# Yusheng-Xu/VGS-SVGS-Segmentation

Measured on AMD Instinct MI355X. Metric: segmented points/sec (end-to-end VGS), higher is better.
Workload: dtype f32

## Files before the change

include/vgs.h:

```cpp
#ifndef VGS_H_
#define VGS_H_

#include <stdint.h>

#ifdef __cplusplus
extern "C" {
#endif

typedef enum {
  VGS_OK = 0,
  VGS_E_ARG = 1,
  VGS_E_STATE = 2,
  VGS_E_HIP = 3,
  VGS_E_NOMEM = 4,
  VGS_E_UNSUPPORTED = 5,
  VGS_E_IO = 6,
  VGS_E_PEER = 7
} vgs_status;

typedef struct {
  int32_t method;
  float voxel_size;
  float graph_size;
  float sig_p, sig_n, sig_o, sig_e, sig_c, sig_w;
// ... 47 lines not shown
vgs_status vgs_commit_points(vgs_ctx* ctx);
vgs_status vgs_host_alloc(void** p, uint64_t bytes);
vgs_status vgs_host_free(void* p);
vgs_status vgs_host_register(void* p, uint64_t bytes);
vgs_status vgs_host_unregister(void* p);

vgs_status vgs_voxelize(vgs_ctx* ctx);
vgs_status vgs_features(vgs_ctx* ctx);
vgs_status vgs_adjacency(vgs_ctx* ctx);
vgs_status vgs_segment(vgs_ctx* ctx);
vgs_status vgs_run(vgs_ctx* ctx);

vgs_status svgs_set_supervoxel_labels(vgs_ctx* ctx, const int32_t* labels_host, int32_t max_label);
vgs_status svgs_supervoxels(vgs_ctx* ctx);
vgs_status svgs_segment(vgs_ctx* ctx);
vgs_status svgs_get_supervoxel_labels(vgs_ctx* ctx, int32_t* labels, int32_t* max_label);

vgs_status vgs_get_counts(vgs_ctx* ctx, int64_t* counts );
vgs_status vgs_get_stage_times(vgs_ctx* ctx, double* ms );
vgs_status vgs_get_schedule_counters(vgs_ctx* ctx, int64_t* out );
vgs_status vgs_get_schedule_counters_ex(vgs_ctx* ctx, int64_t* out, int32_t n);
vgs_status vgs_screen_table(const vgs_params* params, float* d2_stop, float* ctab_scale, float* ctab );
vgs_status vgs_get_bbox(vgs_ctx* ctx, double* min3_max3);
vgs_status vgs_get_voxel_table(vgs_ctx* ctx, uint32_t* key, int32_t* start, int32_t* point_idx);
vgs_status vgs_get_voxel_centers(vgs_ctx* ctx, float* center3V);
vgs_status vgs_get_point_voxel(vgs_ctx* ctx, int32_t* voxel_of_point );
vgs_status vgs_get_attributes(vgs_ctx* ctx, float* centroid, float* normal, float* eigen8, uint8_t* used);
vgs_status vgs_get_lists(vgs_ctx* ctx, int32_t which, int64_t* offsets, int32_t* idx);
enum { VGS_ORDER_VOXEL_ID = 0, VGS_ORDER_REFERENCE = 1 };
vgs_status vgs_get_lists_ordered(vgs_ctx* ctx, int32_t which, int32_t order, int64_t* offsets, int32_t* idx);
vgs_status vgs_get_adjacency_counts(vgs_ctx* ctx, int32_t* n_all );
vgs_status vgs_get_local_weights(vgs_ctx* ctx, int32_t node_id, int32_t* n, int32_t* ids, float* weights);
vgs_status vgs_get_node_labels(vgs_ctx* ctx, int32_t* component_root ,
                               int32_t* kept_label );
vgs_status vgs_get_point_labels(vgs_ctx* ctx, int32_t* labels );
vgs_status vgs_get_point_labels_async(vgs_ctx* ctx, int32_t* labels);
vgs_status vgs_wait_point_labels(vgs_ctx* ctx);
vgs_status vgs_get_point_labels_device(vgs_ctx* ctx, const int32_t** labels_dev );
vgs_status vgs_get_clusters(vgs_ctx* ctx, int64_t* offsets, int32_t* point_idx);
vgs_status vgs_get_clusters_ordered(vgs_ctx* ctx, int32_t order, int64_t* offsets, int32_t* point_idx);
vgs_status vgs_get_clusters_device(vgs_ctx* ctx, const int64_t** offsets_dev, const int32_t** point_idx_dev);
vgs_status vgs_get_segment_descriptors(vgs_ctx* ctx, int64_t* n_points, int32_t* n_nodes, float* bbox6, double* centroid3, double* cov6,
                                       double* evals3, double* evecs9, float* eigen8);
vgs_status vgs_get_segment_descriptors_device(vgs_ctx* ctx, const int64_t** n_points, const int32_t** n_nodes, const float** bbox6,
                                              const double** centroid3, const double** cov6, const double** evals3, const double** evecs9,
                                              const float** eigen8);
// ... 43 lines not shown
```

vgs-svgs-segmentation_amd/_lib.py:

```python
from __future__ import annotations

import ctypes as C
import os
import subprocess

_HERE = os.path.dirname(os.path.abspath(__file__))
LIB_PATH = os.path.join(_HERE, os.path.basename(os.environ.get("VGS_LIB", "libvgs_hip.so")))
CSRC = os.path.join(_HERE, "csrc")

VGS_OK, VGS_E_ARG, VGS_E_STATE, VGS_E_HIP, VGS_E_NOMEM, VGS_E_UNSUPPORTED, VGS_E_IO, VGS_E_PEER = range(8)
STATUS_NAMES = ["VGS_OK", "VGS_E_ARG", "VGS_E_STATE", "VGS_E_HIP", "VGS_E_NOMEM", "VGS_E_UNSUPPORTED", "VGS_E_IO", "VGS_E_PEER"]

N_POINTS, N_FINITE, N_VOXELS, N_USED, N_ADJ, N_CLUSTERS, N_KEPT, N_PAIRS, N_DEPTH, N_ISOLATED, N_REATTACHED, N_SUPERVOXELS = range(12)
N_COUNTS = 16
T_VOXELIZE, T_FEATURES, T_ADJACENCY, T_LOCALCUT, T_MERGE, T_LABELS, T_TOTAL, T_LOCALCUT_KERNEL, T_SUPERVOXEL = range(9)
T_COUNT = 12


class VgsParams(C.Structure):
    _fields_ = [
        ("method", C.c_int32), ("voxel_size", C.c_float), ("graph_size", C.c_float),
        ("sig_p", C.c_float), ("sig_n", C.c_float), ("sig_o", C.c_float), ("sig_e", C.c_float), ("sig_c", C.c_float),
        ("sig_w", C.c_float), ("cut_thred", C.c_float),
        ("points_min", C.c_int32), ("adjacency_min", C.c_int32), ("voxels_min", C.c_int32),
# ... 24 lines not shown
    ("vgs_set_points", C.c_int, [_P, _P, C.c_int64, C.c_int32]),
    ("vgs_set_points_device", C.c_int, [_P, _P, C.c_int64, C.c_int32]),
    ("vgs_stage_points", C.c_int, [_P, _P, C.c_int64, C.c_int32]),
    ("vgs_commit_points", C.c_int, [_P]),
    ("vgs_host_alloc", C.c_int, [C.POINTER(_P), C.c_uint64]),
    ("vgs_host_free", C.c_int, [_P]),
    ("vgs_host_register", C.c_int, [_P, C.c_uint64]),
    ("vgs_host_unregister", C.c_int, [_P]),
    ("vgs_voxelize", C.c_int, [_P]),
    ("vgs_features", C.c_int, [_P]),
    ("vgs_adjacency", C.c_int, [_P]),
    ("vgs_segment", C.c_int, [_P]),
    ("vgs_run", C.c_int, [_P]),
    ("svgs_set_supervoxel_labels", C.c_int, [_P, _P, C.c_int32]),
    ("svgs_supervoxels", C.c_int, [_P]),
    ("svgs_segment", C.c_int, [_P]),
    ("svgs_get_supervoxel_labels", C.c_int, [_P, _P, C.POINTER(C.c_int32)]),
    ("vgs_get_counts", C.c_int, [_P, _P]),
    ("vgs_get_schedule_counters", C.c_int, [_P, _P]),
    ("vgs_get_schedule_counters_ex", C.c_int, [_P, _P, C.c_int32]),
    ("vgs_screen_table", C.c_int, [_P, _P, _P, _P]),
    ("vgs_get_stage_times", C.c_int, [_P, _P]),
    ("vgs_get_bbox", C.c_int, [_P, _P]),
    ("vgs_get_voxel_table", C.c_int, [_P, _P, _P, _P]),
    ("vgs_get_voxel_centers", C.c_int, [_P, _P]),
    ("vgs_get_point_voxel", C.c_int, [_P, _P]),
    ("vgs_get_attributes", C.c_int, [_P, _P, _P, _P, _P]),
    ("vgs_get_lists", C.c_int, [_P, C.c_int32, _P, _P]),
    ("vgs_get_lists_ordered", C.c_int, [_P, C.c_int32, C.c_int32, _P, _P]),
    ("vgs_get_adjacency_counts", C.c_int, [_P, _P]),
    ("vgs_get_local_weights", C.c_int, [_P, C.c_int32, C.POINTER(C.c_int32), _P, _P]),
    ("vgs_get_node_labels", C.c_int, [_P, _P, _P]),
    ("vgs_get_point_labels", C.c_int, [_P, _P]),
    ("vgs_get_point_labels_async", C.c_int, [_P, _P]),
    ("vgs_wait_point_labels", C.c_int, [_P]),
    ("vgs_get_point_labels_device", C.c_int, [_P, C.POINTER(_P)]),
    ("vgs_get_clusters", C.c_int, [_P, _P, _P]),
    ("vgs_get_clusters_ordered", C.c_int, [_P, C.c_int32, _P, _P]),
    ("vgs_get_clusters_device", C.c_int, [_P, _P, _P]),
    ("vgs_get_segment_descriptors", C.c_int, [_P, _P, _P, _P, _P, _P, _P, _P, _P]),
    ("vgs_get_segment_descriptors_device", C.c_int, [_P, _P, _P, _P, _P, _P, _P, _P, _P]),
    ("vgs_get_own_segment_moments", C.c_int, [_P, C.c_int64, _P, _P, _P, _P, _P, _P, _P]),
    ("vgs_segment_descriptors_from_moments", C.c_int, [_P, C.c_int64, _P, _P, _P, _P, _P, _P, _P, _P, _P, _P, _P, _P, _P]),
    ("vgs_get_segment_boxes", C.c_int, [_P, C.c_int32, _P, _P, _P, _P, _P]),
    ("vgs_get_segment_boxes_device", C.c_int, [_P, C.c_int32, _P, _P, _P, _P, _P]),
    ("vgs_get_own_segment_extents", C.c_int, [_P, C.c_int64, C.c_int32, _P, _P, _P, _P, _P, _P, _P]),
# ... 45 lines not shown
```

vgs-svgs-segmentation_amd/api.py:

```python
from __future__ import annotations

import ctypes as C

import numpy as np

from . import _lib
from ._lib import VgsError, VgsGridState, VgsParams


def default_params(method=2, **kw):
    p = VgsParams()
    L = _lib.lib()
    (L.vgs_params_default_svgs if method == 3 else L.vgs_params_default_vgs)(C.byref(p))
    for k, v in kw.items():
        if not hasattr(p, k):
            raise AttributeError(k)
        setattr(p, k, v)
    return p


def parse_task_file(path):
    p = VgsParams()
    a = C.create_string_buffer(512)
    b = C.create_string_buffer(512)
# ... 97 lines not shown
        self._ck(self._L.vgs_get_counts(self._h, _ptr(c)))
        names = ["points", "finite", "voxels", "used", "adj", "clusters", "kept", "pairs", "depth", "isolated", "reattached",
                 "supervoxels", "handed_over", "class_a", "class_bc", "class_d"]
        return {k: int(c[i]) for i, k in enumerate(names)}

    def schedule_counters(self):
        c = np.zeros(13, dtype=np.int64)
        self._ck(self._L.vgs_get_schedule_counters_ex(self._h, _ptr(c), 13))
        names = ("lazy_gave_up", "list_overflow", "handed_over", "dense_sent_on", "handed_over_large", "outside_limits", "cross_put_off", "banded",
                 "extra_large", "pair_list_cut", "pair_list_entries", "voted_over", "pair_list_pool_full")
        return dict(zip(names, (int(x) for x in c)))

    def stage_times(self):
        t = np.zeros(_lib.T_COUNT, dtype=np.float64)
        self._ck(self._L.vgs_get_stage_times(self._h, _ptr(t)))
        names = ["voxelize", "features", "adjacency", "localcut", "merge", "labels", "total", "localcut_kernel", "supervoxel", "localcut_bulk"]
        return {k: float(t[i]) for i, k in enumerate(names)}

    def bbox(self):
        b = np.zeros(6, dtype=np.float64)
        self._ck(self._L.vgs_get_bbox(self._h, _ptr(b)))
        return b

    def voxel_table(self):
        c = self.counts()
        V, nf = c["voxels"], c["finite"]
        key = np.zeros((V, 3), dtype=np.uint32)
        start = np.zeros(V + 1, dtype=np.int32)
        pidx = np.zeros(nf, dtype=np.int32)
        self._ck(self._L.vgs_get_voxel_table(self._h, _ptr(key), _ptr(start), _ptr(pidx)))
        return dict(key=key, start=start, point_idx=pidx)

    def voxel_centers(self):
        V = self.counts()["voxels"]
        c = np.zeros((V, 3), dtype=np.float32)
        self._ck(self._L.vgs_get_voxel_centers(self._h, _ptr(c)))
        return c

    def point_voxel(self):
        out = np.zeros(self.n, dtype=np.int32)
        self._ck(self._L.vgs_get_point_voxel(self._h, _ptr(out)))
        return out

    def attributes(self):
        V = self.counts()["voxels"]
        cen = np.zeros((V, 3), dtype=np.float32)
# ... 328 lines not shown
```

vgs-svgs-segmentation_amd/csrc/capi.hip:

```cpp
#include <algorithm>
#include <cstdio>
#include <cstdlib>
#include <cstring>
#include <fstream>
#include <string>
#include <vector>

#include <dlfcn.h>

#include "vgs_context.hpp"

static thread_local std::string g_create_err;

static const char* const VGS_STAGE_NAMES[VGS_T_COUNT] = {"vgs:voxelize", "vgs:features", "vgs:adjacency", "vgs:localcut", "vgs:merge", "vgs:labels",
                                                         "vgs:total", "vgs:localcut_kernel", "vgs:supervoxels", "vgs:localcut_bulk", "", ""};
struct RoctxApi {
  int (*push)(const char*) = nullptr;
  int (*pop)() = nullptr;
  RoctxApi() {
    for (const char* name : {"librocprofiler-sdk-roctx.so.1", "librocprofiler-sdk-roctx.so", "libroctx64.so.4", "libroctx64.so"}) {
      void* h = dlopen(name, RTLD_LAZY | RTLD_LOCAL);
      if (!h) continue;
      push = (int (*)(const char*))dlsym(h, "roctxRangePushA");
      pop = (int (*)())dlsym(h, "roctxRangePop");
// ... 206 lines not shown
  if (c->ev_ho) (void)hipEventDestroy(c->ev_ho);
  if (c->ev_ho2) (void)hipEventDestroy(c->ev_ho2);
  if (c->ev_d2h) (void)hipEventDestroy(c->ev_d2h);
  delete c;
}

vgs_status vgs_set_params(vgs_ctx* c, const vgs_params* p) {
  if (!c || !p) return VGS_E_ARG;
  if (!(p->voxel_size > 0.f) || !(p->graph_size > 0.f) || !(p->sig_w != 0.f)) { c->err = "vgs_set_params: voxel_size, graph_size > 0, sig_w != 0"; return VGS_E_ARG; }
  if (p->method != c->P.method || p->device != c->P.device) { c->err = "vgs_set_params: method and device are fixed at vgs_create"; return VGS_E_ARG; }
  if (p->vccs_mode != 0 && p->vccs_mode != 1) { c->err = "vgs_set_params: vccs_mode must be 0 (synchronous variant) or 1 (PCL's order)"; return VGS_E_ARG; }
  int keep = ST_SEGMENTED;
  const vgs_params& o = c->P;
  if (p->cut_thred != o.cut_thred || p->sig_p != o.sig_p || p->sig_n != o.sig_n || p->sig_o != o.sig_o || p->sig_e != o.sig_e ||
      p->sig_c != o.sig_c || p->sig_w != o.sig_w || p->adjacency_min != o.adjacency_min || p->voxels_min != o.voxels_min ||
      p->q7_count_as_index != o.q7_count_as_index)
    keep = ST_ADJACENCY;
  if (p->graph_size != o.graph_size) keep = ST_FEATURES;
  if (p->points_min != o.points_min) keep = ST_VOXELS;
  if (p->voxel_size != o.voxel_size || p->seed_size != o.seed_size || p->color_impt != o.color_impt ||
      p->spatial_impt != o.spatial_impt || p->normal_impt != o.normal_impt || p->vccs_mode != o.vccs_mode)
    keep = ST_POINTS;
  if (c->stage > keep) c->stage = keep;
  if (keep < ST_SEGMENTED) { c->sd_valid = false; c->sb_valid[0] = c->sb_valid[1] = false; c->sg_valid = false; c->sg_halo_valid = false; c->sg_own_K = -1; }
  if (keep == ST_POINTS && c->P.method == 3 && !c->sv_labels_external) { c->sv_have_labels = false; c->sv_max_label = 0; c->sv_label_n = -1; }
  c->P = *p;
  return VGS_OK;
}

const char* vgs_last_error_string(const vgs_ctx* c) { return c ? c->err.c_str() : g_create_err.c_str(); }

static vgs_status set_points_common(vgs_ctx* c, int64_t n, int32_t stride_bytes) {
  if (n < 0 || (stride_bytes != 12 && stride_bytes != 16)) { c->err = "set_points: n >= 0 and stride_bytes 12 or 16 required"; return VGS_E_ARG; }
  if (n >= (int64_t)1 << 31) { c->err = "set_points: more than 2^31-1 points"; return VGS_E_UNSUPPORTED; }
  c->N = n;
  c->stride_f = stride_bytes / 4;
  c->stage = ST_POINTS;
  c->sd_valid = false;
  c->sb_valid[0] = c->sb_valid[1] = false;
  c->sg_valid = false; c->sg_halo_valid = false; c->sg_own_K = -1;
  c->grid_covers = false;
  c->counts[VGS_N_POINTS] = n;
  for (int i = 0; i < VGS_T_COUNT; ++i) { c->times[i] = 0; c->tev_pending[i] = false; }
  c->sv_have_labels = false; c->sv_labels_external = false; c->sv_max_label = 0; c->sv_label_n = -1;
  c->n_own = -1; c->own_first = 0;
  return VGS_OK;
// ... 187 lines not shown
    VGS_HIP_TRY(c, hipMemcpy(ev.data(), c->evals.p, ev.size() * 4, hipMemcpyDeviceToHost));
    int64_t tot = 0;
    for (uint32_t x : ev) tot += x;
    c->counts[VGS_N_PAIRS] = tot;
  }
  for (int i = 0; i < VGS_N_COUNTS; ++i) counts[i] = c->counts[i];
  return VGS_OK;
}

vgs_status vgs_get_stage_times(vgs_ctx* c, double* ms) {
  if (!c || !ms) return VGS_E_ARG;
  { vgs_status sr = vgs_resolve_times(c); if (sr != VGS_OK) return sr; }
  if (c->P.method == 2 && c->stage >= ST_SEGMENTED)
    c->times[VGS_T_TOTAL] = c->times[VGS_T_VOXELIZE] + c->times[VGS_T_FEATURES] + c->times[VGS_T_ADJACENCY] + c->times[VGS_T_LOCALCUT] + c->times[VGS_T_MERGE];
  for (int i = 0; i < VGS_T_COUNT; ++i) ms[i] = c->times[i];
  return VGS_OK;
}

vgs_status vgs_get_schedule_counters(vgs_ctx* c, int64_t* out) { return vgs_get_schedule_counters_ex(c, out, 8); }

vgs_status vgs_get_schedule_counters_ex(vgs_ctx* c, int64_t* out, int32_t n) {
  if (!c || !out || n < 0 || n > 16) return VGS_E_ARG;
  for (int i = 0; i < n; ++i) out[i] = c->lc_diag[i];
  return VGS_OK;
}

vgs_status vgs_get_bbox(vgs_ctx* c, double* b) {
  if (!c || !b) return VGS_E_ARG;
  if (c->stage < ST_VOXELS) { c->err = "vgs_get_bbox: voxelize first"; return VGS_E_STATE; }
  for (int a = 0; a < 3; ++a) { b[a] = c->box.min[a]; b[3 + a] = c->box.max[a]; }
  return VGS_OK;
}

vgs_status vgs_get_voxel_table(vgs_ctx* c, uint32_t* key, int32_t* start, int32_t* point_idx) {
  if (!c) return VGS_E_ARG;
  if (c->stage < ST_VOXELS) { c->err = "vgs_get_voxel_table: voxelize first"; return VGS_E_STATE; }
  VGS_HIP_TRY(c, hipSetDevice(c->device));
  if (key && c->V > 0) {
    std::vector<uint64_t> code((size_t)c->V);
    VGS_HIP_TRY(c, hipMemcpy(code.data(), c->vox_code.p, code.size() * 8, hipMemcpyDeviceToHost));
    for (int64_t v = 0; v < c->V; ++v) {
      key[3 * v + 0] = vm_compact21(code[v] >> 2);
      key[3 * v + 1] = vm_compact21(code[v] >> 1);
      key[3 * v + 2] = vm_compact21(code[v]);
    }
  }
// ... 291 lines not shown
```

vgs-svgs-segmentation_amd/csrc/multigpu.hip:

```cpp
#include <algorithm>
#include <cstring>
#include <vector>

#include <rocprim/rocprim.hpp>

#include "vgs_context.hpp"

__global__ void k_point_sources(const uint32_t* __restrict__ perm, const uint32_t* __restrict__ pt_vox, int64_t nf, int64_t own_first, int64_t n_own,
                                int64_t V, uint8_t* __restrict__ mix) {
  int64_t j = (int64_t)blockIdx.x * blockDim.x + threadIdx.x;
  if (j >= nf) return;
  const uint32_t v = pt_vox[j];
  const int64_t i = (int64_t)perm[j];
  if (v != 0xffffffffu) mix[((i >= own_first && i < own_first + n_own) ? 0 : V) + v] = 1;
}

__global__ void k_owned(const uint64_t* __restrict__ vox_code, int64_t V, float res_f, float min_x, float min_y, double lo_x, double lo_y,
                        double hi_x, double hi_y, uint8_t* __restrict__ owned, uint8_t* __restrict__ straddle, const uint8_t* __restrict__ mix, double near) {
  int64_t v = (int64_t)blockIdx.x * blockDim.x + threadIdx.x;
  if (v >= V) return;
  const uint64_t code = vox_code[v];
  const double cx = (double)vm_voxel_center(vm_compact21(code >> 2), res_f, min_x);
  const double cy = (double)vm_voxel_center(vm_compact21(code >> 1), res_f, min_y);
  owned[v] = (cx >= lo_x && cx < hi_x && cy >= lo_y && cy < hi_y) ? 1 : 0;
// ... 237 lines not shown
vgs_status vgs_grid_advance(vgs_ctx* c, vgs_grid_state* g) {
  if (!c || !g) return VGS_E_ARG;
  if (c->stage < ST_POINTS) { c->err = "vgs_grid_advance: no input cloud"; return VGS_E_STATE; }
  VGS_HIP_TRY(c, hipSetDevice(c->device));
  OctreeBox box;
  box_from_state(g, (double)c->P.voxel_size, box);
  const bool was_pinned = c->grid_pinned;
  c->grid_pinned = false;
  vgs_status st = vgs_grow_box_from(c, box, false);
  c->grid_pinned = was_pinned;
  if (st != VGS_OK) return st;
  g->defined = box.defined ? 1 : 0;
  g->depth = box.depth;
  for (int a = 0; a < 3; ++a) { g->min[a] = box.min[a]; g->shift[a] = box.shift[a]; }
  return VGS_OK;
}

vgs_status vgs_set_grid(vgs_ctx* c, const vgs_grid_state* g) {
  if (!c || !g) return VGS_E_ARG;
  if (!g->defined) { c->err = "vgs_set_grid: undefined grid state"; return VGS_E_ARG; }
  box_from_state(g, (double)c->P.voxel_size, c->box);
  c->grid_pinned = true;
  c->grid_covers = false;
  if (c->stage > ST_POINTS) c->stage = ST_POINTS;
  return VGS_OK;
}

vgs_status vgs_set_grid_covering(vgs_ctx* c, const vgs_grid_state* g) {
  vgs_status s = vgs_set_grid(c, g);
  if (s == VGS_OK) c->grid_covers = true;
  return s;
}

vgs_status vgs_set_owned_region(vgs_ctx* c, const double* lo, const double* hi) {
  if (!c || !lo || !hi) return VGS_E_ARG;
  c->own_lo[0] = lo[0]; c->own_lo[1] = lo[1]; c->own_hi[0] = hi[0]; c->own_hi[1] = hi[1];
  c->have_region = true;
  if (c->stage > ST_ADJACENCY) c->stage = ST_ADJACENCY;
  return VGS_OK;
}

vgs_status vgs_set_own_point_range(vgs_ctx* c, int64_t first, int64_t n_own) {
  if (!c || n_own < -1 || first < 0) return VGS_E_ARG;
  c->own_first = first;
  c->n_own = n_own;
  if (c->stage > ST_ADJACENCY) c->stage = ST_ADJACENCY;
// ... 187 lines not shown
```

vgs-svgs-segmentation_amd/csrc/vgs_context.hpp:

```cpp
#ifndef VGS_CONTEXT_HPP_
#define VGS_CONTEXT_HPP_

#include <hip/hip_runtime.h>
#include <stdint.h>
#include <string.h>

#include <string>
#include <vector>

#include "../../include/vgs.h"
#include "vgs_math.h"
#include "pairlist.hpp"

typedef VgsNode NodeRec;
static_assert(sizeof(NodeRec) == 64, "NodeRec must be 64 bytes");

#ifdef __HIPCC__
__device__ __forceinline__ int64_t vgs_xcd_item(unsigned int b, int64_t n) {
  const int64_t per = (n + 7) >> 3;
  return (int64_t)(b & 7u) * per + (int64_t)(b >> 3);
}
#endif
static inline unsigned int vgs_xcd_grid(int64_t n) { return (unsigned int)(((n + 7) >> 3) << 3); }

// ... 90 lines not shown

  const float* xyz = nullptr;
  DevBuf<float> xyz_buf[2];
  int xyz_cur = 0;
  hipStream_t s_h2d = nullptr, s_d2h = nullptr;
  hipEvent_t ev_h2d = nullptr, ev_d2h = nullptr;
  hipEvent_t ev_rb = nullptr;
  bool gathered = false;
  bool bricks_ready = false;
  bool staged = false;
  int64_t staged_n = 0;
  int staged_stride = 12;
  bool pt_labels_pending = false;
  bool labels_event_valid = false;
  bool d2h_open = false;
  const int32_t* d2h_src = nullptr;
  int64_t N = 0;
  int stride_f = 3;

  OctreeBox box;
  bool grid_pinned = false;
  bool grid_covers = false;
  int n_epochs = 0;

  DevBuf<uint64_t> code_a, code_b;
  DevBuf<uint32_t> perm_a, perm_b;
  DevBuf<uint8_t> sort_tmp;
  DevBuf<uint64_t> grow_state;
  DevBuf<uint32_t> pt_vox;
  DevBuf<uint32_t> vox_tile;
  DevBuf<uint32_t> head_flag;
  DevBuf<uint64_t> vox_code;
  DevBuf<uint32_t> vox_start;
  DevBuf<float> xs, ys, zs;
  int64_t Nf = 0;
  int64_t V = 0;
  int code_bits = 0;

  DevBuf<NodeRec> node;
  DevBuf<uint32_t> used_ids, used_rank;
  int64_t U = 0;

  DevBuf<uint64_t> hkey;
  DevBuf<uint32_t> hval;
  uint32_t hbits = 0;
  DevBuf<int32_t> offsets;
// ... 219 lines not shown
```

vgs-svgs-segmentation_amd/csrc/voxelize.hip:

```cpp
#include <cstddef>
#include <cstdlib>
#include <cstring>
#include <string.h>

#include <rocprim/rocprim.hpp>

#include <algorithm>
#include <cmath>
#include <limits>

#include "vgs_context.hpp"

bool OctreeBox::contains(const float* p) const {
  if (!defined) return false;
  for (int a = 0; a < 3; ++a)
    if ((double)p[a] < min[a] || (double)p[a] >= max[a]) return false;
  return true;
}

void OctreeBox::adopt(const float* p) {
  const double eps = (double)std::numeric_limits<float>::epsilon();
  while (true) {
    if (!defined) {
      for (int a = 0; a < 3; ++a) { min[a] = (double)p[a] - res / 2; max[a] = (double)p[a] + res / 2; }
// ... 15 lines not shown
      any = any || hi[a] || ((double)p[a] < min[a]);
    }
    if (!any) return;
    double side = (double)(1u << depth) * res;
    for (int a = 0; a < 3; ++a)
      if (!hi[a]) { min[a] -= side; shift[a] += (1ull << depth); }
    depth++;
    side = (double)(1u << depth) * res - eps;
    for (int a = 0; a < 3; ++a) max[a] = min[a] + side;
  }
}

__device__ __forceinline__ bool finite3(float x, float y, float z) {
  return (vm_bits(x) & 0x7f800000u) != 0x7f800000u && (vm_bits(y) & 0x7f800000u) != 0x7f800000u &&
         (vm_bits(z) & 0x7f800000u) != 0x7f800000u;
}

struct GrowState {
  double min[3], max[3], res;
  unsigned long long shift[3];
  unsigned long long found;
  long long start;
  int depth, defined, done, n_epochs, record, overflow;
  Epoch epochs[VGS_MAX_EPOCHS];
};

struct BoxD { double min[3], max[3]; int defined; };
__device__ __forceinline__ bool fv_outside(float x, float y, float z, const BoxD& g) {
  if (!finite3(x, y, z)) return false;
  return !g.defined || (double)x < g.min[0] || (double)x >= g.max[0] || (double)y < g.min[1] ||
         (double)y >= g.max[1] || (double)z < g.min[2] || (double)z >= g.max[2];
}

__global__ void k_first_violation(const float* __restrict__ xyz, int stride_f, int64_t n, GrowState* __restrict__ gs) {
  if (gs->done) return;
  BoxD box;
  for (int a = 0; a < 3; ++a) { box.min[a] = gs->min[a]; box.max[a] = gs->max[a]; }
  box.defined = gs->defined;
  unsigned long long* result = &gs->found;
  const int64_t start = gs->start;
  unsigned long long best = ~0ull;
  const int64_t tid = (int64_t)blockIdx.x * blockDim.x + threadIdx.x;
  const int64_t nthreads = box.defined ? (int64_t)gridDim.x * blockDim.x : (int64_t)8 * blockDim.x;
  if (tid >= nthreads) return;
  if (stride_f == 3 && (((uintptr_t)xyz) & 15u) == 0) {
    const float4* q = (const float4*)xyz;
// ... 93 lines not shown
    unsigned long long best = ~0ull;
    for (int64_t i = start + tid; i < n_prefix; i += 1024) {
      const float* p = xyz + i * stride_f;
      if (fv_outside(p[0], p[1], p[2], box)) { best = (unsigned long long)i; break; }
    }
    for (int o = 32; o > 0; o >>= 1) { const unsigned long long other = __shfl_down(best, o, 64); best = other < best ? other : best; }
    __syncthreads();
    if ((tid & 63) == 0) s_best[tid >> 6] = best;
    __syncthreads();
    if (tid == 0) {
      unsigned long long b = ~0ull;
      for (int w = 0; w < 16; ++w) b = s_best[w] < b ? s_best[w] : b;
      if (b == ~0ull) { if (S.start < n_prefix) S.start = n_prefix; S.found = ~0ull; s_best[0] = 0ull; }
      else if (pinned) { S.done = 2; s_best[0] = 0ull; }
      else { grow_adopt(xyz, stride_f, &S, b); s_best[0] = (S.done || S.overflow) ? 0ull : 1ull; }
    }
    __syncthreads();
    if (s_best[0] == 0ull) break;
    __syncthreads();
  }
  for (int k = tid; k < (int)(sizeof(GrowState) / 8); k += 1024) ((unsigned long long*)gs)[k] = ((const unsigned long long*)&S)[k];
}

template <typename KeyT>
__global__ void k_make_codes(const float* __restrict__ xyz, int stride_f, int64_t n, const GrowState* __restrict__ gs,
                             double res, int code_bits, KeyT* __restrict__ code, uint32_t* __restrict__ perm, int pack_shift) {
  int64_t i = (int64_t)blockIdx.x * blockDim.x + threadIdx.x;
  if (i >= n) return;
  const float* p = xyz + i * stride_f;
  float x = p[0], y = p[1], z = p[2];
  uint64_t c = 0;
  if (finite3(x, y, z)) {
    int e = gs->n_epochs - 1;
    while (e > 0 && i < gs->epochs[e].first) --e;
    const Epoch& ep = gs->epochs[e];
    uint32_t kx = vm_axis_key(x, ep.min[0], res) + (uint32_t)(gs->shift[0] - ep.shift[0]);
    uint32_t ky = vm_axis_key(y, ep.min[1], res) + (uint32_t)(gs->shift[1] - ep.shift[1]);
    uint32_t kz = vm_axis_key(z, ep.min[2], res) + (uint32_t)(gs->shift[2] - ep.shift[2]);
    c = (1ull << code_bits) | vm_morton(kx, ky, kz);
  }
  if (pack_shift > 0) { code[i] = (KeyT)((c << pack_shift) | (uint64_t)i); return; }
  code[i] = (KeyT)c;
  perm[i] = (uint32_t)i;
}

#define VR_TB 512
#define VR_KPT 4
#define VR_TILE (VR_TB * VR_KPT)

template <typename KeyT>
__device__ __forceinline__ void vr_load(const KeyT* __restrict__ code, int64_t n, int64_t j0, KeyT (&k)[VR_KPT], KeyT& prev) {
  struct alignas(sizeof(KeyT) * VR_KPT) Vec { KeyT v[VR_KPT]; };
  if (j0 + VR_KPT <= n) {
    const Vec q = *(const Vec*)(code + j0);
#pragma unroll
    for (int i = 0; i < VR_KPT; ++i) k[i] = q.v[i];
// ... 102 lines not shown
  if (j0 >= n) return;
  uint32_t out[VR_KPT];
#pragma unroll
  for (int i = 0; i < VR_KPT; ++i) {
    if ((m >> i) & 1u) { vox_code[run] = c[i] & mask; vox_start[run] = (uint32_t)(j0 + i); ++run; }
    out[i] = c[i] != 0 ? run - 1u : 0xffffffffu;
  }
  if (j0 + VR_KPT <= n) {
    *(uint4*)(pt_vox + j0) = make_uint4(out[0], out[1], out[2], out[3]);
  } else {
#pragma unroll
    for (int i = 0; i < VR_KPT; ++i) if (j0 + i < n) pt_vox[j0 + i] = out[i];
  }
}

__global__ void k_gather_points(const float* __restrict__ xyz, int stride_f, const uint32_t* __restrict__ perm, int64_t nf,
                                float* __restrict__ xs, float* __restrict__ ys, float* __restrict__ zs) {
  int64_t j = (int64_t)blockIdx.x * blockDim.x + threadIdx.x;
  if (j >= nf) return;
  const float* p = xyz + (int64_t)perm[j] * stride_f;
  xs[j] = p[0]; ys[j] = p[1]; zs[j] = p[2];
}

vgs_status vgs_grow_box_from(vgs_ctx* c, OctreeBox& box, bool record_epochs) {
  static_assert(sizeof(GrowState) % 8 == 0, "GrowState is copied as 64-bit words");
  VGS_HIP_TRY(c, c->counters.ensure(64));
  VGS_HIP_TRY(c, c->grow_state.ensure(sizeof(GrowState) / 8));
  GrowState* d_g = (GrowState*)c->grow_state.p;
  static thread_local GrowState h;
  std::memset(&h, 0, sizeof(h));
  for (int a = 0; a < 3; ++a) { h.min[a] = box.min[a]; h.max[a] = box.max[a]; h.shift[a] = box.shift[a]; }
  h.res = box.res; h.depth = box.depth; h.defined = box.defined ? 1 : 0;
  h.found = ~0ull; h.start = 0; h.record = record_epochs ? 1 : 0;
  const size_t hb_bytes = offsetof(GrowState, epochs) + sizeof(Epoch);
  const bool covering = c->grid_pinned && c->grid_covers && record_epochs && box.defined;
  if (covering) h.done = 1;
  if (record_epochs && box.defined) {
    Epoch& e = h.epochs[h.n_epochs++];
    e.first = 0;
    for (int a = 0; a < 3; ++a) { e.min[a] = box.min[a]; e.shift[a] = box.shift[a]; }
  }
  {
    const size_t hb = hb_bytes;
    static_assert(offsetof(GrowState, epochs) + sizeof(Epoch) <= 1024, "the growth header fits its slot of the pinned scratch");
    const void* src = &h;
    if (c->pin) { memcpy((char*)c->pin + 1024, &h, hb); src = (char*)c->pin + 1024; }
    VGS_HIP_TRY(c, hipMemcpyAsync(d_g, src, hb, hipMemcpyHostToDevice, c->stream));
  }
  if (covering) {
    c->n_epochs = h.n_epochs;
    return VGS_OK;
  }
  const int pinned = (c->grid_pinned && record_epochs) ? 1 : 0;
  const int blocks = (int)std::max<int64_t>(8, std::min<int64_t>((c->N / 4 + 255) / 256 + 1, (int64_t)c->K.fv_blocks));
  hipLaunchKernelGGL(k_grow_prefix, dim3(1), dim3(1024), 0, c->stream, c->xyz, c->stride_f, std::min<int64_t>(c->N, 8192), d_g, pinned);
  for (int batch = 0; batch < 64; ++batch) {
    for (int k = 0; k < (batch == 0 ? 2 : 8); ++k) {
      hipLaunchKernelGGL(k_first_violation, dim3(blocks), dim3(256), 0, c->stream, c->xyz, c->stride_f, c->N, d_g);
      hipLaunchKernelGGL(k_adopt, dim3(1), dim3(1), 0, c->stream, c->xyz, c->stride_f, d_g, pinned);
    }
    VGS_READBACK(c, &h, d_g, offsetof(GrowState, epochs));
    if (h.done) break;
  }
  if (h.done == 2) { c->err = "a point lies outside the pinned grid"; return VGS_E_ARG; }
  if (h.overflow || !h.done) { c->err = "octree grew more than VGS_MAX_EPOCHS times"; return VGS_E_UNSUPPORTED; }
  for (int a = 0; a < 3; ++a) { box.min[a] = h.min[a]; box.max[a] = h.max[a]; box.shift[a] = h.shift[a]; }
  box.depth = h.depth; box.defined = h.defined != 0;
  if (record_epochs) c->n_epochs = h.n_epochs;
  return VGS_OK;
}

static vgs_status grow_box(vgs_ctx* c) {
  if (!c->grid_pinned) {
    c->box = OctreeBox();
    c->box.res = (double)c->P.voxel_size;
  }
  return vgs_grow_box_from(c, c->box, true);
}

template <typename KeyT>
static vgs_status voxelize_sorted_table(vgs_ctx* c) {
  const int64_t N = c->N;
  const int TB = 256;
  const unsigned nb = (unsigned)((N + TB - 1) / TB);
  KeyT* code_a = (KeyT*)c->code_a.p;
  KeyT* code_b = (KeyT*)c->code_b.p;
  const unsigned key_bits = (unsigned)(c->code_bits + 1);
  int idx_bits = 1;
  while (idx_bits < 32 && ((int64_t)1 << idx_bits) < N) ++idx_bits;
  const int pack_shift = (sizeof(KeyT) == 8 && (int)key_bits + idx_bits <= 64) ? idx_bits : 0;
  hipLaunchKernelGGL((k_make_codes<KeyT>), dim3(nb), dim3(TB), 0, c->stream, c->xyz, c->stride_f, N, (const GrowState*)c->grow_state.p, c->box.res,
                     c->code_bits, code_a, c->perm_a.p, pack_shift);

  using nine_bits = rocprim::radix_sort_config<rocprim::default_config, rocprim::default_config,
                                               rocprim::radix_sort_onesweep_config<rocprim::kernel_config<1024, 6>, rocprim::kernel_config<1024, 6>, 9,
                                                                                   rocprim::block_radix_rank_algorithm::match>>;
  const bool use9 = (key_bits + 8) / 9 < (key_bits + 7) / 8;
  auto sort_pairs = [&](void* tmp, size_t& bytes) -> hipError_t {
    if (pack_shift > 0)
      return use9 ? rocprim::radix_sort_keys_desc<nine_bits>(tmp, bytes, code_a, code_b, (size_t)N, (unsigned)pack_shift, (unsigned)pack_shift + key_bits, c->stream)
                  : rocprim::radix_sort_keys_desc(tmp, bytes, code_a, code_b, (size_t)N, (unsigned)pack_shift, (unsigned)pack_shift + key_bits, c->stream);
    return use9 ? rocprim::radix_sort_pairs_desc<nine_bits>(tmp, bytes, code_a, code_b, c->perm_a.p, c->perm_b.p, (size_t)N, 0, key_bits, c->stream)
                : rocprim::radix_sort_pairs_desc(tmp, bytes, code_a, code_b, c->perm_a.p, c->perm_b.p, (size_t)N, 0, key_bits, c->stream);
  };
  size_t tmp_bytes = 0;
  VGS_HIP_TRY(c, sort_pairs(nullptr, tmp_bytes));
  VGS_HIP_TRY(c, c->sort_tmp.ensure(tmp_bytes));
  VGS_HIP_TRY(c, sort_pairs(c->sort_tmp.p, tmp_bytes));
  const int64_t n_tiles = (N + VR_TILE - 1) / VR_TILE;
  VGS_HIP_TRY(c, c->vox_tile.ensure((size_t)(2 * n_tiles)));
  uint32_t* tile_heads = c->vox_tile.p;
  uint32_t* tile_valid = c->vox_tile.p + n_tiles;
  unsigned long long* d_cnt = (unsigned long long*)c->counters.p;
  hipLaunchKernelGGL((k_run_counts<KeyT>), dim3((unsigned)n_tiles), dim3(VR_TB), 0, c->stream, code_b, N, pack_shift, c->perm_b.p, tile_heads, tile_valid);
  hipLaunchKernelGGL(k_tile_offsets, dim3(1), dim3(1024), 0, c->stream, tile_heads, tile_valid, n_tiles, d_cnt);
  unsigned long long h2[2] = {0, 0};
  if (vgs_can_split_readback(c)) {
    { vgs_status sb = vgs_readback_begin(c, d_cnt, sizeof(h2)); if (sb != VGS_OK) return sb; }
    VGS_HIP_TRY(c, c->xs.ensure(N + 1)); VGS_HIP_TRY(c, c->ys.ensure(N + 1)); VGS_HIP_TRY(c, c->zs.ensure(N + 1));
    hipLaunchKernelGGL(k_gather_points, dim3(nb), dim3(TB), 0, c->stream, c->xyz, c->stride_f, c->perm_b.p, N, c->xs.p, c->ys.p, c->zs.p);
    c->gathered = true;
    { vgs_status se = vgs_readback_end(c, h2, sizeof(h2)); if (se != VGS_OK) return se; }
  } else {
    VGS_READBACK(c, h2, d_cnt, sizeof(h2));
  }
  const unsigned long long nf = h2[0];
  const uint32_t v_total = (uint32_t)h2[1];
  c->Nf = (int64_t)nf;
  c->V = (int64_t)v_total;
  VGS_HIP_TRY(c, c->vox_code.ensure(c->V + 1)); VGS_HIP_TRY(c, c->vox_start.ensure(c->V + 1));
  const uint64_t mask = (c->code_bits >= 64) ? ~0ull : ((1ull << c->code_bits) - 1ull);
  hipLaunchKernelGGL((k_voxel_runs<KeyT>), dim3((unsigned)n_tiles), dim3(VR_TB), 0, c->stream, code_b, N, pack_shift, tile_heads, mask, c->pt_vox.p,
                     c->vox_code.p, c->vox_start.p, v_total, (uint32_t)c->Nf);
  return VGS_OK;
}

vgs_status vgs_stage_voxelize(vgs_ctx* c) {
  const int64_t N = c->N;
  c->V = 0; c->Nf = 0; c->U = 0;
  vgs_status st = grow_box(c);
  if (st != VGS_OK) return st;
  if (c->n_epochs == 0) {
    c->counts[VGS_N_FINITE] = 0; c->counts[VGS_N_VOXELS] = 0; c->counts[VGS_N_DEPTH] = 0;
    return VGS_OK;
  }
  if (c->box.depth > 21) { c->err = "octree depth > 21 (64-bit voxel codes exhausted)"; return VGS_E_UNSUPPORTED; }
  c->code_bits = 3 * c->box.depth;

  VGS_HIP_TRY(c, c->code_a.ensure(N)); VGS_HIP_TRY(c, c->code_b.ensure(N));
  VGS_HIP_TRY(c, c->perm_a.ensure(N)); VGS_HIP_TRY(c, c->perm_b.ensure(N));
  VGS_HIP_TRY(c, c->pt_vox.ensure(N));
  const int TB = 256;
  c->gathered = false;
  st = (c->code_bits + 1 <= 32) ? voxelize_sorted_table<uint32_t>(c) : voxelize_sorted_table<uint64_t>(c);
  if (st != VGS_OK) return st;
  if (!c->gathered) { VGS_HIP_TRY(c, c->xs.ensure(c->Nf + 1)); VGS_HIP_TRY(c, c->ys.ensure(c->Nf + 1)); VGS_HIP_TRY(c, c->zs.ensure(c->Nf + 1)); }
  if (c->Nf > 0 && !c->gathered) {
    const unsigned nbf = (unsigned)((c->Nf + TB - 1) / TB);
    hipLaunchKernelGGL(k_gather_points, dim3(nbf), dim3(TB), 0, c->stream, c->xyz, c->stride_f, c->perm_b.p, c->Nf, c->xs.p, c->ys.p,
                       c->zs.p);
  }
  VGS_HIP_TRY(c, hipGetLastError());
  c->counts[VGS_N_FINITE] = c->Nf;
  c->counts[VGS_N_VOXELS] = c->V;
  c->counts[VGS_N_DEPTH] = c->box.depth;
  return VGS_OK;
}
```

Measured before the change: 1.636 billion.

## Speculatively voxelize with cached octree depth to skip box-growth readback

Remembers the octree depth from the previous voxelization and, on the next run, grows the box from only a point prefix, then generates codes, sorts and builds runs at the hinted depth without waiting for full box growth. A checked code kernel flags any point outside the box or any depth mismatch, and one combined readback of the growth header validates the speculation. On a miss it falls back to the full checked path. This removes a host-device synchronisation and the full growth pass per run, at the risk of redoing the work when point extents change between calls.

```diff
diff --git a/include/vgs.h b/include/vgs.h
--- a/include/vgs.h
+++ b/include/vgs.h
@@ -93,6 +93,8 @@
 vgs_status vgs_get_schedule_counters_ex(vgs_ctx* ctx, int64_t* out, int32_t n);
 vgs_status vgs_screen_table(const vgs_params* params, float* d2_stop, float* ctab_scale, float* ctab );
 vgs_status vgs_get_bbox(vgs_ctx* ctx, double* min3_max3);
+enum { VGS_VOXPATH_CHECKED = 0, VGS_VOXPATH_SPECULATIVE = 1, VGS_VOXPATH_FALLBACK = 2 };
+vgs_status vgs_get_voxelize_info(vgs_ctx* ctx, int64_t* out );
 vgs_status vgs_get_voxel_table(vgs_ctx* ctx, uint32_t* key, int32_t* start, int32_t* point_idx);
 vgs_status vgs_get_voxel_centers(vgs_ctx* ctx, float* center3V);
 vgs_status vgs_get_point_voxel(vgs_ctx* ctx, int32_t* voxel_of_point );
diff --git a/vgs-svgs-segmentation_amd/_lib.py b/vgs-svgs-segmentation_amd/_lib.py
--- a/vgs-svgs-segmentation_amd/_lib.py
+++ b/vgs-svgs-segmentation_amd/_lib.py
@@ -70,6 +70,7 @@
     ("vgs_screen_table", C.c_int, [_P, _P, _P, _P]),
     ("vgs_get_stage_times", C.c_int, [_P, _P]),
     ("vgs_get_bbox", C.c_int, [_P, _P]),
+    ("vgs_get_voxelize_info", C.c_int, [_P, _P]),
     ("vgs_get_voxel_table", C.c_int, [_P, _P, _P, _P]),
     ("vgs_get_voxel_centers", C.c_int, [_P, _P]),
     ("vgs_get_point_voxel", C.c_int, [_P, _P]),
diff --git a/vgs-svgs-segmentation_amd/api.py b/vgs-svgs-segmentation_amd/api.py
--- a/vgs-svgs-segmentation_amd/api.py
+++ b/vgs-svgs-segmentation_amd/api.py
@@ -143,6 +143,12 @@
         self._ck(self._L.vgs_get_bbox(self._h, _ptr(b)))
         return b
 
+    def voxelize_info(self):
+        o = np.zeros(8, dtype=np.int64)
+        self._ck(self._L.vgs_get_voxelize_info(self._h, _ptr(o)))
+        return dict(path=("checked", "speculative", "fallback")[int(o[0])], depth=int(o[1]), shift=tuple(int(x) for x in o[2:5]),
+                    epochs=int(o[5]), depth_hint=int(o[6]))
+
     def voxel_table(self):
         c = self.counts()
         V, nf = c["voxels"], c["finite"]
diff --git a/vgs-svgs-segmentation_amd/csrc/capi.hip b/vgs-svgs-segmentation_amd/csrc/capi.hip
--- a/vgs-svgs-segmentation_amd/csrc/capi.hip
+++ b/vgs-svgs-segmentation_amd/csrc/capi.hip
@@ -252,6 +252,7 @@
       p->spatial_impt != o.spatial_impt || p->normal_impt != o.normal_impt || p->vccs_mode != o.vccs_mode)
     keep = ST_POINTS;
   if (c->stage > keep) c->stage = keep;
+  if (p->voxel_size != o.voxel_size) c->depth_hint = 0;
   if (keep < ST_SEGMENTED) { c->sd_valid = false; c->sb_valid[0] = c->sb_valid[1] = false; c->sg_valid = false; c->sg_halo_valid = false; c->sg_own_K = -1; }
   if (keep == ST_POINTS && c->P.method == 3 && !c->sv_labels_external) { c->sv_have_labels = false; c->sv_max_label = 0; c->sv_label_n = -1; }
   c->P = *p;
@@ -485,6 +486,15 @@
 vgs_status vgs_get_schedule_counters_ex(vgs_ctx* c, int64_t* out, int32_t n) {
   if (!c || !out || n < 0 || n > 16) return VGS_E_ARG;
   for (int i = 0; i < n; ++i) out[i] = c->lc_diag[i];
+  return VGS_OK;
+}
+
+vgs_status vgs_get_voxelize_info(vgs_ctx* c, int64_t* out) {
+  if (!c || !out) return VGS_E_ARG;
+  if (c->stage < ST_VOXELS) { c->err = "vgs_get_voxelize_info: voxelize first"; return VGS_E_STATE; }
+  out[0] = c->vox_path; out[1] = c->box.defined ? c->box.depth : 0;
+  for (int a = 0; a < 3; ++a) out[2 + a] = (int64_t)c->box.shift[a];
+  out[5] = c->n_epochs; out[6] = c->depth_hint; out[7] = 0;
   return VGS_OK;
 }
 
diff --git a/vgs-svgs-segmentation_amd/csrc/multigpu.hip b/vgs-svgs-segmentation_amd/csrc/multigpu.hip
--- a/vgs-svgs-segmentation_amd/csrc/multigpu.hip
+++ b/vgs-svgs-segmentation_amd/csrc/multigpu.hip
@@ -283,6 +283,7 @@
   box_from_state(g, (double)c->P.voxel_size, c->box);
   c->grid_pinned = true;
   c->grid_covers = false;
+  c->depth_hint = 0;
   if (c->stage > ST_POINTS) c->stage = ST_POINTS;
   return VGS_OK;
 }
diff --git a/vgs-svgs-segmentation_amd/csrc/vgs_context.hpp b/vgs-svgs-segmentation_amd/csrc/vgs_context.hpp
--- a/vgs-svgs-segmentation_amd/csrc/vgs_context.hpp
+++ b/vgs-svgs-segmentation_amd/csrc/vgs_context.hpp
@@ -136,6 +136,8 @@
   bool grid_pinned = false;
   bool grid_covers = false;
   int n_epochs = 0;
+  int depth_hint = 0;
+  int vox_path = 0;
 
   DevBuf<uint64_t> code_a, code_b;
   DevBuf<uint32_t> perm_a, perm_b;
diff --git a/vgs-svgs-segmentation_amd/csrc/voxelize.hip b/vgs-svgs-segmentation_amd/csrc/voxelize.hip
--- a/vgs-svgs-segmentation_amd/csrc/voxelize.hip
+++ b/vgs-svgs-segmentation_amd/csrc/voxelize.hip
@@ -61,6 +61,8 @@
   unsigned long long found;
   long long start;
   int depth, defined, done, n_epochs, record, overflow;
+  unsigned long long cnt[2];
+  unsigned int spec_miss, spec_pad;
   Epoch epochs[VGS_MAX_EPOCHS];
 };
 
@@ -200,16 +202,25 @@
   for (int k = tid; k < (int)(sizeof(GrowState) / 8); k += 1024) ((unsigned long long*)gs)[k] = ((const unsigned long long*)&S)[k];
 }
 
-template <typename KeyT>
+template <typename KeyT, bool CHECKED>
 __global__ void k_make_codes(const float* __restrict__ xyz, int stride_f, int64_t n, const GrowState* __restrict__ gs,
-                             double res, int code_bits, KeyT* __restrict__ code, uint32_t* __restrict__ perm, int pack_shift) {
+                             double res, int code_bits, KeyT* __restrict__ code, uint32_t* __restrict__ perm, int pack_shift,
+                             int depth_hint, unsigned int* __restrict__ miss) {
   int64_t i = (int64_t)blockIdx.x * blockDim.x + threadIdx.x;
   if (i >= n) return;
   const float* p = xyz + i * stride_f;
   float x = p[0], y = p[1], z = p[2];
+  if (CHECKED) {
+    BoxD box;
+    for (int a = 0; a < 3; ++a) { box.min[a] = gs->min[a]; box.max[a] = gs->max[a]; }
+    box.defined = gs->defined;
+    if (i >= gs->start && fv_outside(x, y, z, box)) *miss = 1u;
+    if (i == 0 && (gs->depth != depth_hint || gs->done || gs->overflow)) *miss = 1u;
+  }
   uint64_t c = 0;
   if (finite3(x, y, z)) {
     int e = gs->n_epochs - 1;
+    if (CHECKED && e < 0) e = 0;
     while (e > 0 && i < gs->epochs[e].first) --e;
     const Epoch& ep = gs->epochs[e];
     uint32_t kx = vm_axis_key(x, ep.min[0], res) + (uint32_t)(gs->shift[0] - ep.shift[0]);
@@ -358,18 +369,17 @@
   xs[j] = p[0]; ys[j] = p[1]; zs[j] = p[2];
 }
 
-vgs_status vgs_grow_box_from(vgs_ctx* c, OctreeBox& box, bool record_epochs) {
+static vgs_status grow_start(vgs_ctx* c, const OctreeBox& box, bool record_epochs, GrowState& h, bool& covering) {
   static_assert(sizeof(GrowState) % 8 == 0, "GrowState is copied as 64-bit words");
   VGS_HIP_TRY(c, c->counters.ensure(64));
   VGS_HIP_TRY(c, c->grow_state.ensure(sizeof(GrowState) / 8));
   GrowState* d_g = (GrowState*)c->grow_state.p;
-  static thread_local GrowState h;
   std::memset(&h, 0, sizeof(h));
   for (int a = 0; a < 3; ++a) { h.min[a] = box.min[a]; h.max[a] = box.max[a]; h.shift[a] = box.shift[a]; }
   h.res = box.res; h.depth = box.depth; h.defined = box.defined ? 1 : 0;
   h.found = ~0ull; h.start = 0; h.record = record_epochs ? 1 : 0;
   const size_t hb_bytes = offsetof(GrowState, epochs) + sizeof(Epoch);
-  const bool covering = c->grid_pinned && c->grid_covers && record_epochs && box.defined;
+  covering = c->grid_pinned && c->grid_covers && record_epochs && box.defined;
   if (covering) h.done = 1;
   if (record_epochs && box.defined) {
     Epoch& e = h.epochs[h.n_epochs++];
@@ -383,6 +393,14 @@
     if (c->pin) { memcpy((char*)c->pin + 1024, &h, hb); src = (char*)c->pin + 1024; }
     VGS_HIP_TRY(c, hipMemcpyAsync(d_g, src, hb, hipMemcpyHostToDevice, c->stream));
   }
+  return VGS_OK;
+}
+
+vgs_status vgs_grow_box_from(vgs_ctx* c, OctreeBox& box, bool record_epochs) {
+  static thread_local GrowState h;
+  bool covering = false;
+  { vgs_status ss = grow_start(c, box, record_epochs, h, covering); if (ss != VGS_OK) return ss; }
+  GrowState* d_g = (GrowState*)c->grow_state.p;
   if (covering) {
     c->n_epochs = h.n_epochs;
     return VGS_OK;
@@ -415,7 +433,7 @@
 }
 
 template <typename KeyT>
-static vgs_status voxelize_sorted_table(vgs_ctx* c) {
+static vgs_status voxelize_sorted_table(vgs_ctx* c, int spec_depth = 0, bool* spec_ok = nullptr) {
   const int64_t N = c->N;
   const int TB = 256;
   const unsigned nb = (unsigned)((N + TB - 1) / TB);
@@ -425,8 +443,13 @@
   int idx_bits = 1;
   while (idx_bits < 32 && ((int64_t)1 << idx_bits) < N) ++idx_bits;
   const int pack_shift = (sizeof(KeyT) == 8 && (int)key_bits + idx_bits <= 64) ? idx_bits : 0;
-  hipLaunchKernelGGL((k_make_codes<KeyT>), dim3(nb), dim3(TB), 0, c->stream, c->xyz, c->stride_f, N, (const GrowState*)c->grow_state.p, c->box.res,
-                     c->code_bits, code_a, c->perm_a.p, pack_shift);
+  GrowState* d_g = (GrowState*)c->grow_state.p;
+  if (spec_depth > 0)
+    hipLaunchKernelGGL((k_make_codes<KeyT, true>), dim3(nb), dim3(TB), 0, c->stream, c->xyz, c->stride_f, N, (const GrowState*)d_g, c->box.res,
+                       c->code_bits, code_a, c->perm_a.p, pack_shift, spec_depth, &d_g->spec_miss);
+  else
+    hipLaunchKernelGGL((k_make_codes<KeyT, false>), dim3(nb), dim3(TB), 0, c->stream, c->xyz, c->stride_f, N, (const GrowState*)d_g, c->box.res,
+                       c->code_bits, code_a, c->perm_a.p, pack_shift, 0, (unsigned int*)nullptr);
 
   using nine_bits = rocprim::radix_sort_config<rocprim::default_config, rocprim::default_config,
                                                rocprim::radix_sort_onesweep_config<rocprim::kernel_config<1024, 6>, rocprim::kernel_config<1024, 6>, 9,
@@ -447,11 +470,26 @@
   VGS_HIP_TRY(c, c->vox_tile.ensure((size_t)(2 * n_tiles)));
   uint32_t* tile_heads = c->vox_tile.p;
   uint32_t* tile_valid = c->vox_tile.p + n_tiles;
-  unsigned long long* d_cnt = (unsigned long long*)c->counters.p;
+  unsigned long long* d_cnt = spec_depth > 0 ? d_g->cnt : (unsigned long long*)c->counters.p;
   hipLaunchKernelGGL((k_run_counts<KeyT>), dim3((unsigned)n_tiles), dim3(VR_TB), 0, c->stream, code_b, N, pack_shift, c->perm_b.p, tile_heads, tile_valid);
   hipLaunchKernelGGL(k_tile_offsets, dim3(1), dim3(1024), 0, c->stream, tile_heads, tile_valid, n_tiles, d_cnt);
   unsigned long long h2[2] = {0, 0};
-  if (vgs_can_split_readback(c)) {
+  if (spec_depth > 0) {
+    static thread_local GrowState h;
+    const size_t hb = offsetof(GrowState, epochs);
+    static_assert(offsetof(GrowState, epochs) <= 2048, "the growth header fits the split read-back's half of the pinned scratch");
+    { vgs_status sb = vgs_readback_begin(c, d_g, hb); if (sb != VGS_OK) return sb; }
+    VGS_HIP_TRY(c, c->xs.ensure(N + 1)); VGS_HIP_TRY(c, c->ys.ensure(N + 1)); VGS_HIP_TRY(c, c->zs.ensure(N + 1));
+    hipLaunchKernelGGL(k_gather_points, dim3(nb), dim3(TB), 0, c->stream, c->xyz, c->stride_f, c->perm_b.p, N, c->xs.p, c->ys.p, c->zs.p);
+    c->gathered = true;
+    { vgs_status se = vgs_readback_end(c, &h, hb); if (se != VGS_OK) return se; }
+    *spec_ok = !h.spec_miss && !h.done && !h.overflow && h.defined && h.n_epochs > 0 && h.depth == spec_depth;
+    if (!*spec_ok) return VGS_OK;
+    for (int a = 0; a < 3; ++a) { c->box.min[a] = h.min[a]; c->box.max[a] = h.max[a]; c->box.shift[a] = h.shift[a]; }
+    c->box.depth = h.depth; c->box.defined = true;
+    c->n_epochs = h.n_epochs;
+    h2[0] = h.cnt[0]; h2[1] = h.cnt[1];
+  } else if (vgs_can_split_readback(c)) {
     { vgs_status sb = vgs_readback_begin(c, d_cnt, sizeof(h2)); if (sb != VGS_OK) return sb; }
     VGS_HIP_TRY(c, c->xs.ensure(N + 1)); VGS_HIP_TRY(c, c->ys.ensure(N + 1)); VGS_HIP_TRY(c, c->zs.ensure(N + 1));
     hipLaunchKernelGGL(k_gather_points, dim3(nb), dim3(TB), 0, c->stream, c->xyz, c->stride_f, c->perm_b.p, N, c->xs.p, c->ys.p, c->zs.p);
@@ -471,25 +509,50 @@
   return VGS_OK;
 }
 
-vgs_status vgs_stage_voxelize(vgs_ctx* c) {
+static vgs_status voxelize_keys(vgs_ctx* c, int spec_depth = 0, bool* spec_ok = nullptr) {
   const int64_t N = c->N;
-  c->V = 0; c->Nf = 0; c->U = 0;
-  vgs_status st = grow_box(c);
-  if (st != VGS_OK) return st;
-  if (c->n_epochs == 0) {
-    c->counts[VGS_N_FINITE] = 0; c->counts[VGS_N_VOXELS] = 0; c->counts[VGS_N_DEPTH] = 0;
-    return VGS_OK;
-  }
-  if (c->box.depth > 21) { c->err = "octree depth > 21 (64-bit voxel codes exhausted)"; return VGS_E_UNSUPPORTED; }
-  c->code_bits = 3 * c->box.depth;
-
   VGS_HIP_TRY(c, c->code_a.ensure(N)); VGS_HIP_TRY(c, c->code_b.ensure(N));
   VGS_HIP_TRY(c, c->perm_a.ensure(N)); VGS_HIP_TRY(c, c->perm_b.ensure(N));
   VGS_HIP_TRY(c, c->pt_vox.ensure(N));
+  c->gathered = false;
+  return (c->code_bits + 1 <= 32) ? voxelize_sorted_table<uint32_t>(c, spec_depth, spec_ok) : voxelize_sorted_table<uint64_t>(c, spec_depth, spec_ok);
+}
+
+static vgs_status voxelize_speculative(vgs_ctx* c, int depth_hint, bool* ok) {
+  static thread_local GrowState h;
+  c->box = OctreeBox();
+  c->box.res = (double)c->P.voxel_size;
+  bool covering = false;
+  { vgs_status ss = grow_start(c, c->box, true, h, covering); if (ss != VGS_OK) return ss; }
+  hipLaunchKernelGGL(k_grow_prefix, dim3(1), dim3(1024), 0, c->stream, c->xyz, c->stride_f, std::min<int64_t>(c->N, 8192), (GrowState*)c->grow_state.p, 0);
+  c->code_bits = 3 * depth_hint;
+  return voxelize_keys(c, depth_hint, ok);
+}
+
+vgs_status vgs_stage_voxelize(vgs_ctx* c) {
+  c->V = 0; c->Nf = 0; c->U = 0;
+  const int hint = c->depth_hint;
+  c->depth_hint = 0;
+  c->vox_path = VGS_VOXPATH_CHECKED;
+  bool done = false;
+  if (hint > 0 && !c->grid_pinned && c->N > 0 && vgs_can_split_readback(c)) {
+    vgs_status ss = voxelize_speculative(c, hint, &done);
+    if (ss != VGS_OK) return ss;
+    c->vox_path = done ? VGS_VOXPATH_SPECULATIVE : VGS_VOXPATH_FALLBACK;
+  }
+  if (!done) {
+    vgs_status st = grow_box(c);
+    if (st != VGS_OK) return st;
+    if (c->n_epochs == 0) {
+      c->counts[VGS_N_FINITE] = 0; c->counts[VGS_N_VOXELS] = 0; c->counts[VGS_N_DEPTH] = 0;
+      return VGS_OK;
+    }
+    if (c->box.depth > 21) { c->err = "octree depth > 21 (64-bit voxel codes exhausted)"; return VGS_E_UNSUPPORTED; }
+    c->code_bits = 3 * c->box.depth;
+    st = voxelize_keys(c);
+    if (st != VGS_OK) return st;
+  }
   const int TB = 256;
-  c->gathered = false;
-  st = (c->code_bits + 1 <= 32) ? voxelize_sorted_table<uint32_t>(c) : voxelize_sorted_table<uint64_t>(c);
-  if (st != VGS_OK) return st;
   if (!c->gathered) { VGS_HIP_TRY(c, c->xs.ensure(c->Nf + 1)); VGS_HIP_TRY(c, c->ys.ensure(c->Nf + 1)); VGS_HIP_TRY(c, c->zs.ensure(c->Nf + 1)); }
   if (c->Nf > 0 && !c->gathered) {
     const unsigned nbf = (unsigned)((c->Nf + TB - 1) / TB);
@@ -500,5 +563,6 @@
   c->counts[VGS_N_FINITE] = c->Nf;
   c->counts[VGS_N_VOXELS] = c->V;
   c->counts[VGS_N_DEPTH] = c->box.depth;
+  if (!c->grid_pinned) c->depth_hint = c->box.depth;
   return VGS_OK;
 }
```

Measured after the change: 1.645 billion, median of 6. No clear change (+0.5%).
